# dremovd/PPO

Measured on AMD Instinct MI355X. Metric: env-steps/sec (Pong-shaped synthetic, 256 envs/GPU), higher is better.
Workload: dtype f32

## Files before the change

include/ppo_amd.h:

```cpp
#ifndef PPO_AMD_H
#define PPO_AMD_H

#include <stddef.h>
#include <stdint.h>

#ifdef __cplusplus
extern "C" {
#endif

#define PPO_OK 0
#define PPO_E_INVALID (-1)
#define PPO_E_HIP (-2)
#define PPO_E_ALIGN (-3)

#define PPO_TERM_NONE 0
#define PPO_TERM_U8 1
#define PPO_TERM_F32 2

#define PPO_SCAN_AUTO 0
#define PPO_SCAN_COLUMNS 1
#define PPO_SCAN_TILES 2

int ppo_version(void);
const char *ppo_last_error(void);
// ... 63 lines not shown
    float *dweight;
    float *dbias;
    int n_slabs, cin, cout;
    int accumulate;
} ppo_wgrad_job;
int ppo_conv3x3_backward_weight_slabs_f32(const void *in, int in_mode, const float *dy, void *workspace,
                                          size_t workspace_bytes, int n, int cin, int cout, int h, int w,
                                          int *n_slabs, void *stream);
int ppo_conv3x3_backward_weight_slabs_batch_f32(const void *const *ins, int in_mode, const float *const *dys,
                                                void *const *workspaces, size_t workspace_bytes, int count, int n, int cin,
                                                int cout, int h, int w, int *n_slabs, void *stream);
int ppo_conv3x3_backward_weight_slabs_batch_mixed_f32(const void *const *ins, const int *relu, const float *const *dys,
                                                      void *const *workspaces, size_t workspace_bytes, int count, int n,
                                                      int cin, int cout, int h, int w, int *n_slabs, void *stream);
int ppo_conv3x3_backward_weight_bf16x3_supported(int cin, int cout, int h, int w);
int ppo_conv3x3_backward_weight_slabs_batch_bf16x3(const float *const *ins, const int *relu, const float *const *dys,
                                                   void *const *workspaces, size_t workspace_bytes, int count, int n, int cin,
                                                   int cout, int h, int w, int *n_slabs, void *stream);
int ppo_conv3x3_backward_weight_pooled_supported(int cin, int cout, int h, int w);
int ppo_conv3x3_backward_weight_slabs_pooled_f32(const void *in, int in_mode, const float *g, const uint8_t *argmax,
                                                 void *workspace, size_t workspace_bytes, int n, int cin, int cout, int h,
                                                 int w, int *n_slabs, void *stream);
int ppo_conv3x3_wgrad_reduce_f32(const ppo_wgrad_job *jobs, int n_jobs, void *stream);

int ppo_maxpool3x3s2_forward_f32(const float *in, float *out, uint8_t *argmax, int n, int c, int h, int w,
                                 void *stream);
int ppo_maxpool3x3s2_backward_f32(const float *dout, const uint8_t *argmax, float *din, int n, int c, int h, int w,
                                  void *stream);

size_t ppo_gemm_workspace_bytes(int M, int N, int K);
int ppo_gemm_f32(const float *A, int64_t a_sm, int64_t a_sk, int relu_a, const float *B, int64_t b_sk, int64_t b_sn,
                 int relu_b, const float *bias, const float *mask, float *C, int64_t ldc, int M, int N, int K,
                 void *workspace, size_t workspace_bytes, void *stream);

int ppo_dense_heads_forward_f32(const float *x, int relu_x, const float *W, const float *b, const float *Wh, const float *bh,
                                int relu_h, float *h, float *heads, int M, int K, int H, int NH, void *workspace,
                                size_t workspace_bytes, void *stream);

int ppo_dense_heads_act_forward_f32(const float *x, int relu_x, const float *W, const float *b, const float *Wh,
                                    const float *bh, int relu_h, float *h, float *heads, int M, int K, int H, int NH,
                                    void *workspace, size_t workspace_bytes, int n_actions, float temperature,
                                    uint64_t seed, uint64_t offset, float *log_policy, int32_t *actions, float *log_pac,
                                    float *raw_policy, float *values, int n_value_heads, void *stream);
int ppo_dense_heads_loss_forward_f32(const float *x, int relu_x, const float *W, const float *b, const float *Wh, const float *bh,
                                     int relu_h, float *h, float *heads, int M, int K, int H, int NH, void *workspace,
                                     size_t workspace_bytes, int n_actions, int n_value_heads, const int32_t *actions,
                                     const float *old_log_pac, const float *old_log_policy, const float *advantages,
                                     const float *returns, float eps_clip, float ent_coef, float vf_coef, float grad_scale,
                                     float *dheads, float *stats, const int32_t *index, void *stream);

int ppo_heads_backward_f32(const float *dheads, const float *hin, int relu_in, const float *gate, const float *Wh, float *dh,
                           float *dWh, float *dbh, float *db_next, int B, int H, int NH, void *stream);
int ppo_colsum_f32(const float *X, int M, int N, int64_t ldx, float *out, int accumulate, void *stream);

int ppo_policy_act_f32(const float *heads, int B, int ldo, int n_actions, float temperature, const float *uniform,
                       uint64_t seed, uint64_t offset, int greedy, float *log_policy, int32_t *actions,
                       float *log_pac, float *raw_policy, float *values, int n_value_heads, void *stream);

int ppo_ppo_loss_f32(const float *heads, int B, int ldo, int n_actions, int n_value_heads, const int32_t *actions,
                     const float *old_log_pac, const float *old_log_policy, const float *advantages,
                     const float *returns, float eps_clip, float ent_coef, float vf_coef, float grad_scale,
                     float *dheads, float *stats, const int32_t *index, void *stream);

int ppo_tanh_forward_f32(const float *x, float *y, size_t n, void *stream);
int ppo_tanh_backward_f32(const float *dy, const float *y, float *dx, size_t n, void *stream);

int ppo_value_loss_f32(const float *heads, int B, int ldo, int value_col, int n_value_heads, const float *returns,
                       float vf_coef, int tvf_col, int n_tvf, int tvf_stride, const float *tvf_returns,
                       const float *tvf_weights, float tvf_coef, float grad_scale, float *dheads, float *stats,
                       const int32_t *index, float tvf_keep_prob, uint64_t seed, uint64_t offset, void *stream);

int ppo_distil_loss_f32(const float *heads, int B, int ldo, int n_actions, int pred_col, int n_pred, int pred_stride,
                        int vector_targets, const float *targets, const float *weights, const float *old_policy,
                        const float *log_std, float beta, float grad_scale, float *dheads, float *stats,
                        const int32_t *index, void *stream);

int ppo_gaussian_act_f32(const float *heads, int B, int ldo, int n_actions, const float *log_std, const float *normal,
                         uint64_t seed, uint64_t offset, int deterministic, float *actions, float *log_pac,
                         float *raw_policy, float *values, int n_value_heads, void *stream);

int ppo_gaussian_loss_f32(const float *heads, int B, int ldo, int n_actions, int n_value_heads, const float *actions,
                          const float *old_log_pac, const float *advantages, const float *returns,
                          const float *log_std, float eps_clip, float vf_coef, float grad_scale, float *dheads,
                          float *dlog_std_rows, float *stats, const int32_t *index, void *stream);

size_t ppo_adam_workspace_bytes(void);
int ppo_adam_step_f32(float *params, const float *grads, float *exp_avg, float *exp_avg_sq, int64_t n, int64_t step,
                      double lr, double beta1, double beta2, double eps, float max_grad_norm, float grad_div,
                      void *workspace, float *grad_norm_out, void *stream);
int ppo_adam_step_presummed_f32(float *params, const float *grads, float *exp_avg, float *exp_avg_sq, int64_t n,
                                int64_t step, double lr, double beta1, double beta2, double eps, float max_grad_norm,
                                float grad_div, const float *partials, int n_partials, float *grad_norm_out, void *stream);
int ppo_adam_step_scatter_f32(float *params, const float *grads, float *exp_avg, float *exp_avg_sq, int64_t n, int64_t step,
                              double lr, double beta1, double beta2, double eps, float max_grad_norm, float grad_div,
                              void *workspace, float *grad_norm_out, const int32_t *scatter, int64_t n_scatter,
                              float *packed, void *stream);

int ppo_gather_rows(const void *src, int64_t row_bytes, int64_t n_src_rows, const int32_t *index, int n_rows,
                    void *dst, void *stream);

size_t ppo_moments_workspace_bytes(void);
int ppo_moments_f64(const float *x, int64_t n, double *moments, void *workspace, void *stream);
int ppo_normalize_f32(const float *x, int64_t n, const double *moments, float eps, float *out, float *mean_std_out,
                      void *stream);
int ppo_accumulate_f32(float *dst, const float *src, int64_t n, void *stream);
int ppo_mask_mul_f32(float *w, const uint8_t *mask, int64_t n, void *stream);
// ... 141 lines not shown
```

ppo_amd/_lib.py:

```python
import ctypes
import os
import threading

HERE = os.path.dirname(os.path.abspath(__file__))
LIB_PATH = os.environ.get("PPO_AMD_LIB") or os.path.join(HERE, "lib", "libppo_amd.so")

PPO_TERM_NONE, PPO_TERM_U8, PPO_TERM_F32 = 0, 1, 2
PPO_SCAN_AUTO, PPO_SCAN_COLUMNS, PPO_SCAN_TILES = 0, 1, 2
PPO_IN_NONE, PPO_IN_RELU, PPO_IN_U8 = 0, 1, 2

_vp = ctypes.c_void_p
_i = ctypes.c_int
_i64 = ctypes.c_int64
_d = ctypes.c_double
_f = ctypes.c_float
_sz = ctypes.c_size_t
_u64 = ctypes.c_uint64

SIGNATURES = {
    "ppo_version": (_i, []),
    "ppo_last_error": (ctypes.c_char_p, []),
    "ppo_gae_scan_f32": (_i, [_vp, _vp, _vp, _vp, _i, _vp, _vp, _i, _i, _i64, _d, _d, _d, _i, _vp]),
    "ppo_bootstrapped_returns_f32": (_i, [_vp, _vp, _i, _vp, _vp, _d, _vp, _i, _i, _i64, _vp]),
    "ppo_conv3x3_forward_f32": (_i, [_vp, _i, _vp, _vp, _vp, _vp, _i, _i, _i, _i, _i, _vp]),
    "ppo_conv3x3_backward_data_f32": (_i, [_vp, _vp, _vp, _vp, _vp, _i, _i, _i, _i, _i, _vp]),
    "ppo_conv3x3_wgrad_workspace_bytes": (_sz, [_i, _i]),
    "ppo_conv3x3_backward_weight_f32": (_i, [_vp, _i, _vp, _vp, _vp, _vp, _sz, _i, _i, _i, _i, _i, _i, _vp]),
    "ppo_maxpool3x3s2_forward_f32": (_i, [_vp, _vp, _vp, _i, _i, _i, _i, _vp]),
    "ppo_maxpool3x3s2_backward_f32": (_i, [_vp, _vp, _vp, _i, _i, _i, _i, _vp]),
    "ppo_gemm_workspace_bytes": (_sz, [_i, _i, _i]),
    "ppo_gemm_f32": (_i, [_vp, _i64, _i64, _i, _vp, _i64, _i64, _i, _vp, _vp, _vp, _i64, _i, _i, _i, _vp, _sz, _vp]),
    "ppo_colsum_f32": (_i, [_vp, _i, _i, _i64, _vp, _i, _vp]),
    "ppo_heads_backward_f32": (_i, [_vp, _vp, _i, _vp, _vp, _vp, _vp, _vp, _vp, _i, _i, _i, _vp]),
    "ppo_dense_heads_forward_f32": (_i, [_vp, _i, _vp, _vp, _vp, _vp, _i, _vp, _vp, _i, _i, _i, _i, _vp, _sz, _vp]),
    "ppo_dense_heads_act_forward_f32": (_i, [_vp, _i, _vp, _vp, _vp, _vp, _i, _vp, _vp, _i, _i, _i, _i, _vp, _sz, _i, _f, _u64,
                                             _u64, _vp, _vp, _vp, _vp, _vp, _i, _vp]),
    "ppo_dense_heads_loss_forward_f32": (_i, [_vp, _i, _vp, _vp, _vp, _vp, _i, _vp, _vp, _i, _i, _i, _i, _vp, _sz, _i, _i, _vp, _vp, _vp,
                                              _vp, _vp, _f, _f, _f, _f, _vp, _vp, _vp, _vp]),
    "ppo_policy_act_f32": (_i, [_vp, _i, _i, _i, _f, _vp, _u64, _u64, _i, _vp, _vp, _vp, _vp, _vp, _i, _vp]),
    "ppo_gather_rows": (_i, [_vp, _i64, _i64, _vp, _i, _vp, _vp]),
    "ppo_moments_workspace_bytes": (_sz, []),
    "ppo_moments_f64": (_i, [_vp, _i64, _vp, _vp, _vp]),
    "ppo_normalize_f32": (_i, [_vp, _i64, _vp, _f, _vp, _vp, _vp]),
    "ppo_accumulate_f32": (_i, [_vp, _vp, _i64, _vp]),
    "ppo_mask_mul_f32": (_i, [_vp, _vp, _i64, _vp]),
    "ppo_tvf_returns_workspace_bytes": (_sz, [_i, _i, _i, _i, _i]),
    "ppo_tvf_returns_f32": (_i, [_vp, _vp, _vp, _i, _i, _i, _i, _i, _d, _vp, _vp, _vp, _i, _i, _vp, _vp, _vp, _vp, _vp,
                                 _vp, _sz, _vp, _vp]),
    "ppo_synth_env_create": (_vp, [_i, _i64, _u64, _d, _i64, _i]),
    "ppo_synth_env_destroy": (None, [_vp]),
    "ppo_synth_env_reset": (_i, [_vp, _vp]),
    "ppo_synth_env_step": (_i, [_vp, _vp, _vp, _vp, _vp, _vp, _vp, _vp]),
    "ppo_synth_env_step_upload": (_i, [_vp, _vp, _vp, _vp, _vp, _vp, _vp, _vp, _vp, _i, _vp]),
    "ppo_synth_env_get_state": (_i, [_vp, _vp, _vp, _vp]),
    "ppo_synth_env_set_state": (_i, [_vp, _vp, _vp, _vp, _vp]),
    "ppo_ppo_loss_f32": (_i, [_vp, _i, _i, _i, _i, _vp, _vp, _vp, _vp, _vp, _f, _f, _f, _f, _vp, _vp, _vp, _vp]),
    "ppo_conv3x3_pool_forward_f32": (_i, [_vp, _i, _vp, _vp, _vp, _vp, _i, _i, _i, _i, _i, _vp]),
    "ppo_conv3x3_packed_floats": (_sz, [_i, _i, _i]),
    "ppo_conv3x3_pack_weights_f32": (_i, [_vp, _i, _vp]),
    "ppo_conv3x3_forward_packed_f32": (_i, [_vp, _i, _vp, _vp, _vp, _vp, _i, _i, _i, _i, _i, _vp]),
    "ppo_conv3x3_backward_data_packed_f32": (_i, [_vp, _vp, _vp, _vp, _vp, _i, _i, _i, _i, _i, _vp]),
    "ppo_conv3x3_pool_forward_packed_f32": (_i, [_vp, _i, _vp, _vp, _vp, _vp, _i, _i, _i, _i, _i, _vp]),
    "ppo_conv3x3_pool_forward_packed_indexed_f32": (_i, [_vp, _vp, _i, _vp, _vp, _vp, _vp, _i, _i, _i, _i, _i, _vp]),
    "ppo_conv1_pool_form": (_i, [_i]),
    "ppo_conv3x3_block_supported": (_i, [_i, _i, _i]),
    "ppo_conv3x3_block_forward_packed_f32": (_i, [_vp, _vp, _vp, _vp, _vp, _vp, _i, _i, _i, _i, _vp]),
    "ppo_conv3x3_backward_weight_slabs_f32": (_i, [_vp, _i, _vp, _vp, _sz, _i, _i, _i, _i, _i, _vp, _vp]),
    "ppo_conv3x3_backward_weight_pooled_supported": (_i, [_i, _i, _i, _i]),
    "ppo_conv3x3_backward_weight_slabs_pooled_f32": (_i, [_vp, _i, _vp, _vp, _vp, _sz, _i, _i, _i, _i, _i, _vp, _vp]),
    "ppo_conv3x3_backward_weight_slabs_pooled_indexed_f32": (_i, [_vp, _vp, _i, _vp, _vp, _vp, _sz, _i, _i, _i, _i, _i, _vp, _vp]),
    "ppo_conv3x3_backward_weight_slabs_batch_f32": (_i, [_vp, _i, _vp, _vp, _sz, _i, _i, _i, _i, _i, _i, _vp, _vp]),
    "ppo_conv3x3_backward_weight_slabs_batch_mixed_f32": (_i, [_vp, _vp, _vp, _vp, _sz, _i, _i, _i, _i, _i, _i, _vp, _vp]),
    "ppo_conv3x3_backward_weight_bf16x3_supported": (_i, [_i, _i, _i, _i]),
    "ppo_conv3x3_backward_weight_slabs_batch_bf16x3": (_i, [_vp, _vp, _vp, _vp, _sz, _i, _i, _i, _i, _i, _i, _vp, _vp]),
    "ppo_conv3x3_wgrad_reduce_f32": (_i, [_vp, _i, _vp]),
    "ppo_tanh_forward_f32": (_i, [_vp, _vp, _sz, _vp]),
    "ppo_tanh_backward_f32": (_i, [_vp, _vp, _vp, _sz, _vp]),
    "ppo_value_loss_f32": (_i, [_vp, _i, _i, _i, _i, _vp, _f, _i, _i, _i, _vp, _vp, _f, _f, _vp, _vp, _vp, _f, _u64, _u64, _vp]),
    "ppo_distil_loss_f32": (_i, [_vp, _i, _i, _i, _i, _i, _i, _i, _vp, _vp, _vp, _vp, _f, _f, _vp, _vp, _vp, _vp]),
    "ppo_gaussian_act_f32": (_i, [_vp, _i, _i, _i, _vp, _vp, _u64, _u64, _i, _vp, _vp, _vp, _vp, _i, _vp]),
    "ppo_gaussian_loss_f32": (_i, [_vp, _i, _i, _i, _i, _vp, _vp, _vp, _vp, _vp, _f, _f, _f, _vp, _vp, _vp, _vp, _vp]),
    "ppo_impala_stack_tail_supported": (_i, [_i, _i, _i]),
    "ppo_impala_stack_tail_forward_f32": (_i, [_vp, _vp, _vp, _vp, _vp, _vp, _vp, _i, _i, _i, _i, _vp]),
    "ppo_impala_stack_full_supported": (_i, [_i, _i, _i]),
    "ppo_impala_stack_full_backward_f32": (_i, [_vp] * 10 + [_i, _i, _i, _i, _vp]),
    "ppo_impala_stack_chain_forward_f32": (_i, [_vp] * 15 + [_i, _i, _i, _i, _vp]),
# ... 136 lines not shown
```

ppo_amd/csrc/gemm.hip:

```cpp
#include <algorithm>

#include "common.h"
#include "loss_rows.h"
#include "policy_act.h"
#include "mfma.h"

namespace ppo {
namespace {

#ifndef PPO_TUNE_GEMM_BK
#define PPO_TUNE_GEMM_BK 32
#endif
constexpr int BM = 64, BN = 64, BK = PPO_TUNE_GEMM_BK;
constexpr int PITCH_M = 80, PITCH_K = BK + 2;
constexpr int TILE_WORDS = BM * PITCH_K > BK * PITCH_M ? BM * PITCH_K : BK * PITCH_M;

struct GemmArgs {
    const float *A;
    const float *B;
    float *C;
    const float *bias;
    const float *mask;
    int M, N, K;
    int64_t a_sm, a_sk, b_sk, b_sn, ldc;
// ... 77 lines not shown
};
__device__ __forceinline__ TileId tile_of(int id, int gm, int gn, int split)
{
    const int xcd = id % kXcds, slot = id / kXcds;
    TileId t;
    if (split > 1) {
        const int per = (split + kXcds - 1) / kXcds;
        t.z = xcd * per + slot % per;
        const int tile = slot / per;
        t.tn = tile % gn;
        t.tm = tile / gn;
        t.live = t.z < split && t.tm < gm;
    } else if (gn >= gm) {
        t.z = 0;
        t.tm = slot % gm;
        t.tn = xcd + kXcds * (slot / gm);
        t.live = t.tn < gn;
    } else {
        t.z = 0;
        t.tn = slot % gn;
        t.tm = xcd + kXcds * (slot / gn);
        t.live = t.tm < gm;
    }
    return t;
}
inline int tile_grid(int gm, int gn, int split)
{
    if (split > 1) return kXcds * ((split + kXcds - 1) / kXcds) * gm * gn;
    const int lo = gn >= gm ? gm : gn, hi = gn >= gm ? gn : gm;
    return kXcds * ((hi + kXcds - 1) / kXcds) * lo;
}

#ifndef PPO_TUNE_GEMM_DEPTH
#define PPO_TUNE_GEMM_DEPTH 4
#endif
constexpr int DEPTH = PPO_TUNE_GEMM_DEPTH;

#ifdef PPO_TUNE_GEMM_STAMPS
__device__ unsigned long long ppo_gemm_stamps[1024 * 8];
#define PPO_GSTAMP(slot)                                                                          \
    do {                                                                                          \
        unsigned long long t_;                                                                    \
        __builtin_amdgcn_sched_barrier(0);                                                        \
        asm volatile("s_memtime %0\n\ts_waitcnt lgkmcnt(0)" : "=s"(t_)::"memory");               \
        __builtin_amdgcn_sched_barrier(0);                                                        \
        if (threadIdx.x == 0 && blockIdx.x < 1024) ppo_gemm_stamps[blockIdx.x * 8 + (slot)] = t_; \
    } while (0)
#else
#define PPO_GSTAMP(slot)
#endif
static_assert(DEPTH % 2 == 0, "the LDS buffer of a slab is its slot's parity");

template <bool a_kfast, bool b_kfast, bool vec>
__global__ __launch_bounds__(kGemmThreads) void gemm_f32_kernel(GemmArgs p, int gm, int gn)
{
    __shared__ __align__(16) float s_a[2][TILE_WORDS];
    __shared__ __align__(16) float s_b[2][TILE_WORDS];
    const TileId t = tile_of(blockIdx.x, gm, gn, p.split);
    if (!t.live) return;
    const int tid = threadIdx.x;
    const int lane = tid & 63;
    const int wave = tid >> 6;
    const int l15 = lane & 15;
    const int g = lane >> 4;
    const int wm = (wave / (BN / kWaveN)) * 32;
    const int wn = (wave % (BN / kWaveN)) * kWaveN;
    const int m0 = t.tm * BM;
    const int n0 = t.tn * BN;
    const int kbeg = t.z * p.k_per_slice;
    const int kend = min(p.K, kbeg + p.k_per_slice);

    f32x4 acc[2][kNJ];
#pragma unroll
    for (int i = 0; i < 2; ++i)
#pragma unroll
        for (int j = 0; j < kNJ; ++j) acc[i][j] = f32x4{0.f, 0.f, 0.f, 0.f};

    const int nslabs = kbeg < kend ? (kend - kbeg + BK - 1) / BK : 0;
    const int ngroups = (nslabs + DEPTH - 1) / DEPTH;
    const __amdgpu_buffer_rsrc_t bufA = operand_rsrc(p.A), bufB = operand_rsrc(p.B);
    Slab ra[DEPTH], rb[DEPTH];

    auto fetch = [&](int d, int slab) {
        slab_load<a_kfast, vec>(ra[d], bufA, (int)p.a_sm, (int)p.a_sk, m0, p.M, kbeg + slab * BK, kend, tid);
        slab_load<b_kfast, vec>(rb[d], bufB, (int)p.b_sn, (int)p.b_sk, n0, p.N, kbeg + slab * BK, kend, tid);
    };
    auto stage = [&](int d) {
        slab_store(ra[d], s_a[d & 1], a_kfast, p.relu_a, tid);
        slab_store(rb[d], s_b[d & 1], b_kfast, p.relu_b, tid);
        __syncthreads();
    };
    auto multiply = [&](int d) {
        const float *sa = s_a[d & 1], *sb = s_b[d & 1];
        float a[BK / 4][2], b[BK / 4][kNJ];
#pragma unroll
        for (int ks = 0; ks < BK / 4; ++ks) {
#pragma unroll
            for (int i = 0; i < 2; ++i)
                a[ks][i] = a_kfast ? sa[(wm + i * 16 + l15) * PITCH_K + ks * 4 + g]
                                   : sa[(ks * 4 + g) * PITCH_M + wm + i * 16 + l15];
#pragma unroll
            for (int j = 0; j < kNJ; ++j)
                b[ks][j] = b_kfast ? sb[(wn + j * 16 + l15) * PITCH_K + ks * 4 + g]
                                   : sb[(ks * 4 + g) * PITCH_M + wn + j * 16 + l15];
        }
        __builtin_amdgcn_sched_barrier(0);
#pragma unroll
        for (int ks = 0; ks < BK / 4; ++ks)
#pragma unroll
            for (int i = 0; i < 2; ++i)
#pragma unroll
                for (int j = 0; j < kNJ; ++j) acc[i][j] = mfma16(a[ks][i], b[ks][j], acc[i][j]);
// ... 39 lines not shown
            for (int q = 0; q < kPasses; ++q) {
                const int m = m0 + row0 + kRowsPerPass * q;
                const int off = (m < p.M && col_in) ? (m * (int)p.ldc + n0 + col) * 4 : kOutside;
                gate[q] = buffer_f32x4(bufM, off);
            }
        }
        if (finish && p.bias && col_in) bias4 = *reinterpret_cast<const float4 *>(p.bias + n0 + col);
        __syncthreads();
#pragma unroll
        for (int i = 0; i < 2; ++i)
#pragma unroll
            for (int j = 0; j < kNJ; ++j)
#pragma unroll
                for (int r = 0; r < 4; ++r)
                    sc[(wm + i * 16 + g * 4 + r) * PITCH_C + wn + j * 16 + l15] = acc[i][j][r];
        __syncthreads();
#pragma unroll
        for (int q = 0; q < kPasses; ++q) {
            const int row = row0 + kRowsPerPass * q, m = m0 + row;
            float4 v = *reinterpret_cast<const float4 *>(sc + row * PITCH_C + col);
            if (finish) {
                v.x += bias4.x, v.y += bias4.y, v.z += bias4.z, v.w += bias4.w;
                if (p.mask) {
                    v.x = gate[q].x > 0.f ? v.x : 0.f;
                    v.y = gate[q].y > 0.f ? v.y : 0.f;
                    v.z = gate[q].z > 0.f ? v.z : 0.f;
                    v.w = gate[q].w > 0.f ? v.w : 0.f;
                }
            }
            if (m < p.M && col_in) *reinterpret_cast<float4 *>(C + m * ldc + n0 + col) = v;
        }
    } else {
#pragma unroll
        for (int i = 0; i < 2; ++i)
#pragma unroll
            for (int j = 0; j < kNJ; ++j)
#pragma unroll
                for (int r = 0; r < 4; ++r) {
                    const int m = m0 + wm + i * 16 + g * 4 + r;
                    const int n = n0 + wn + j * 16 + l15;
                    if (m < p.M && n < p.N) {
                        float v = acc[i][j][r];
                        if (finish) {
                            if (p.bias) v += p.bias[n];
                            if (p.mask) v = p.mask[m * p.ldc + n] > 0.f ? v : 0.f;
                        }
                        C[m * ldc + n] = v;
                    }
                }
    }
    PPO_GSTAMP(4);
}

__global__ __launch_bounds__(256) void gemm_finalize_kernel(const float *__restrict__ partial, int split, int M, int N,
                                                            const float *__restrict__ bias,
                                                            const float *__restrict__ mask, float *__restrict__ C,
                                                            int64_t ldc)
{
    const int idx = blockIdx.x * blockDim.x + threadIdx.x;
    if (idx >= M * N) return;
    const int m = idx / N, n = idx % N;
    float v = 0.f;
    const size_t stride = (size_t)M * N;
    int s = 0;
    for (; s + 8 <= split; s += 8) {
        float t[8];
#pragma unroll
        for (int u = 0; u < 8; ++u) t[u] = partial[(size_t)(s + u) * stride + idx];
#pragma unroll
        for (int u = 0; u < 8; ++u) v += t[u];
    }
    for (; s < split; ++s) v += partial[(size_t)s * stride + idx];
    if (bias) v += bias[n];
    if (mask) v = mask[m * ldc + n] > 0.f ? v : 0.f;
    C[m * ldc + n] = v;
}

constexpr int kRowsMaxN = 32, kRowsMaxKPerLane = 8;

template <int NB, int KPL>
__global__ __launch_bounds__(256) void gemm_rows_kernel(GemmArgs p)
{
    const int lane = threadIdx.x & 63;
    const int m = blockIdx.x * 4 + __builtin_amdgcn_readfirstlane(threadIdx.x >> 6);
    if (m >= p.M) return;
    const __amdgpu_buffer_rsrc_t bufA = operand_rsrc(p.A), bufB = operand_rsrc(p.B);
    bool kin[KPL];
#pragma unroll
    for (int i = 0; i < KPL; ++i) kin[i] = lane + 64 * i < p.K;
    float av[KPL];
#pragma unroll
    for (int i = 0; i < KPL; ++i) {
        const int off = kin[i] ? (m * (int)p.a_sm + lane + 64 * i) * 4 : kOutside;
        av[i] = buffer_f32(bufA, off);
    }
    for (int n0 = 0; n0 < p.N; n0 += NB) {
        float bv[NB][KPL];
#pragma unroll
        for (int j = 0; j < NB; ++j) {
            const int row = min(n0 + j, p.N - 1) * (int)p.b_sn;
#pragma unroll
            for (int i = 0; i < KPL; ++i) {
                const int off = kin[i] ? (row + lane + 64 * i) * 4 : kOutside;
                bv[j][i] = buffer_f32(bufB, off);
            }
        }
// ... 21 lines not shown
            if (p.mask) v = p.mask[m * p.ldc + n] > 0.f ? v : 0.f;
            p.C[m * p.ldc + n] = v;
        }
    }
}

__global__ __launch_bounds__(256) void gemm_small_kernel(GemmArgs p)
{
    __shared__ float s[256];
    const int o = blockIdx.x * 16 + (threadIdx.x & 15);
    const int part = threadIdx.x >> 4;
    const bool live = o < p.M * p.N;
    const int m = live ? o / p.N : 0, n = live ? o - m * p.N : 0;
    const float *a = p.A + m * p.a_sm;
    const float *b = p.B + n * p.b_sn;
    const int per = (p.K + 15) / 16;
    const int k0 = part * per, k1 = min(p.K, k0 + per);
    float acc = 0.f;
    if (live) {
        int k = k0;
        for (; k + 8 <= k1; k += 8) {
            float av[8], bv[8];
#pragma unroll
            for (int u = 0; u < 8; ++u) {
                av[u] = a[(k + u) * p.a_sk];
                bv[u] = b[(k + u) * p.b_sk];
            }
#pragma unroll
            for (int u = 0; u < 8; ++u) {
                if (p.relu_a) av[u] = fmaxf(av[u], 0.f);
                if (p.relu_b) bv[u] = fmaxf(bv[u], 0.f);
                acc = fmaf(av[u], bv[u], acc);
            }
        }
        for (; k < k1; ++k) {
            float a0 = a[k * p.a_sk], b0 = b[k * p.b_sk];
            if (p.relu_a) a0 = fmaxf(a0, 0.f);
            if (p.relu_b) b0 = fmaxf(b0, 0.f);
            acc = fmaf(a0, b0, acc);
        }
    }
    s[threadIdx.x] = acc;
    __syncthreads();
    if (part == 0 && live) {
        float v = 0.f;
#pragma unroll
        for (int q = 0; q < 16; ++q) v += s[q * 16 + threadIdx.x];
        if (p.bias) v += p.bias[n];
        if (p.mask) v = p.mask[m * p.ldc + n] > 0.f ? v : 0.f;
        p.C[m * p.ldc + n] = v;
    }
}

__global__ __launch_bounds__(256) void colsum_kernel(const float *__restrict__ X, int M, int N, int64_t ldx,
                                                     float *__restrict__ out, int accumulate)
{
    __shared__ float s[256];
    const int n = blockIdx.x * 16 + (threadIdx.x & 15);
    const int part = threadIdx.x >> 4;
    float v = 0.f;
    if (n < N) {
        for (int m = part; m < M; m += 16 * 8) {
            float t[8];
#pragma unroll
            for (int u = 0; u < 8; ++u) {
                const int mm = m + 16 * u;
                t[u] = mm < M ? X[mm * ldx + n] : 0.f;
            }
#pragma unroll
            for (int u = 0; u < 8; ++u) v += t[u];
        }
    }
    s[threadIdx.x] = v;
    __syncthreads();
    if (part == 0 && n < N) {
        float t = 0.f;
#pragma unroll
        for (int q = 0; q < 16; ++q) t += s[q * 16 + threadIdx.x];
        out[n] = accumulate ? out[n] + t : t;
    }
}

struct ActTail {
    float temperature;
    uint64_t seed, offset;
    ActOut out;
    int loss;
    PpoLossP lp;
    float *dheads;
    const int32_t *index;
};

template <int KPL, int NA, int NHT>
__global__ __launch_bounds__(256) void finalize_heads_kernel(const float *__restrict__ partial, int split, int M, int H,
                                                            const float *__restrict__ bias, float *__restrict__ h,
                                                            const float *__restrict__ Wh, const float *__restrict__ bh, int NH,
                                                            int relu_h, float *__restrict__ heads, ActTail act)
{
    const int lane = threadIdx.x & 63;
    const int m = blockIdx.x * 4 + __builtin_amdgcn_readfirstlane(threadIdx.x >> 6);
    if (m >= M) return;
    const __amdgpu_buffer_rsrc_t pb = buffer_of(partial), wb = buffer_of(Wh), bb = buffer_of(bias, bias != nullptr);
    const int stride = M * H;
    int off[KPL];
#pragma unroll
    for (int i = 0; i < KPL; ++i) off[i] = lane + 64 * i < H ? m * H + lane + 64 * i : -1;
    float bv[NHT][KPL];
#pragma unroll
    for (int j = 0; j < NHT; ++j) {
        const int row = min(j, NH - 1) * H;
#pragma unroll
        for (int i = 0; i < KPL; ++i) bv[j][i] = buffer_f32(wb, off[i] < 0 ? kOutside : (row + lane + 64 * i) * 4);
    }
    float hv[KPL];
#pragma unroll
    for (int i = 0; i < KPL; ++i) hv[i] = 0.f;
    float bsv[KPL];
#pragma unroll
    for (int i = 0; i < KPL; ++i) bsv[i] = buffer_f32(bb, off[i] < 0 ? kOutside : (lane + 64 * i) * 4);
    int s = 0;
    for (; s + 16 <= split; s += 16) {
        float t[KPL][16];
#pragma unroll
        for (int i = 0; i < KPL; ++i)
#pragma unroll
            for (int u = 0; u < 16; ++u) t[i][u] = buffer_f32(pb, off[i] < 0 ? kOutside : ((s + u) * stride + off[i]) * 4);
#pragma unroll
        for (int i = 0; i < KPL; ++i)
#pragma unroll
            for (int u = 0; u < 16; ++u) hv[i] += t[i][u];
    }
    for (; s + 8 <= split; s += 8) {
// ... 125 lines not shown
    }
#pragma unroll
    for (int j = 0; j < 16; ++j) s_red[j][tid] = dW[j];
    s_red[16][tid] = dbn;
    s_red[17][tid] = dbj;
    __syncthreads();
    if (part == 0) {
        float tot[18];
#pragma unroll
        for (int v = 0; v < 18; ++v) {
            float t = 0.f;
#pragma unroll
            for (int q = 0; q < 16; ++q) t += s_red[v][q * 16 + kk];
            tot[v] = t;
        }
        if (col) {
#pragma unroll
            for (int j = 0; j < 16; ++j)
                if (j < a.NH) a.dWh[j * a.H + k] = tot[j];
            if (a.db_next) a.db_next[k] = tot[16];
        }
        if ((int)blockIdx.x == a.xb && a.dbh && kk < a.NH) a.dbh[kk] = tot[17];
    }
}

inline bool vec_ok(const float *P, int64_t s_tile, int64_t s_k, int tile_extent, int k_extent)
{
    const int64_t other = s_k == 1 ? s_tile : s_k;
    const int extent = s_k == 1 ? k_extent : tile_extent;
    return (s_k == 1 || s_tile == 1) && other % 4 == 0 && extent % 4 == 0 && aligned(P, 16);
}

}
}

extern "C" size_t ppo_gemm_workspace_bytes(int M, int N, int K)
{
    (void)K;
    return (size_t)32 * M * N * sizeof(float);
}

namespace ppo {
namespace {
struct HeadsTail {
    const float *Wh, *bh;
    float *heads;
    int NH, relu_h;
    bool fused;
    const ActTail *act = nullptr;
    int act_n = 0;
    bool act_fused = false;
};

int gemm_dispatch(const float *A, int64_t a_sm, int64_t a_sk, int relu_a, const float *B, int64_t b_sk, int64_t b_sn,
                  int relu_b, const float *bias, const float *mask, float *C, int64_t ldc, int M, int N, int K,
                  void *workspace, size_t workspace_bytes, void *stream, HeadsTail *tail)
{
    if (M < 0 || N < 0 || K < 0) return fail(PPO_E_INVALID, "ppo_gemm_f32: negative dimension");
    if (M == 0 || N == 0) return PPO_OK;
    if (!A || !B || !C) return fail(PPO_E_INVALID, "ppo_gemm_f32: null pointer");
    if (ldc < N) return fail(PPO_E_INVALID, "ppo_gemm_f32: ldc < N");
    const int64_t a_last = (int64_t)(M - 1) * a_sm + (int64_t)(K - 1) * a_sk, b_last = (int64_t)(N - 1) * b_sn + (int64_t)(K - 1) * b_sk;
    if (K > 0 && (a_last * 4 + 16 > (int64_t)kBufferBytes || b_last * 4 + 16 > (int64_t)kBufferBytes || a_sm < 0 || a_sk < 0 ||
                  b_sn < 0 || b_sk < 0))
        return fail(PPO_E_INVALID, "ppo_gemm_f32: operand spans 2 GiB or more (or a negative stride); split the batch");
    hipStream_t st = as_stream(stream);
    if ((N <= 16 || K <= 16 || (M <= 16 && a_sm == 1)) && (int64_t)M * N <= (1 << 22)) {
        GemmArgs q{A, B, C, bias, mask, M, N, K, a_sm, a_sk, b_sk, b_sn, ldc, relu_a, relu_b, K, 1, 0, 0, 0};
        if (N <= kRowsMaxN && a_sk == 1 && b_sk == 1 && K <= 64 * kRowsMaxKPerLane) {
            if (K <= 256 && N <= 16)
                hipLaunchKernelGGL((gemm_rows_kernel<16, 4>), dim3((M + 3) / 4), dim3(256), 0, st, q);
            else if (K <= 256)
                hipLaunchKernelGGL((gemm_rows_kernel<8, 4>), dim3((M + 3) / 4), dim3(256), 0, st, q);
            else
                hipLaunchKernelGGL((gemm_rows_kernel<4, kRowsMaxKPerLane>), dim3((M + 3) / 4), dim3(256), 0, st, q);
            return check_launch("gemm_rows_kernel");
        }
        hipLaunchKernelGGL(gemm_small_kernel, dim3((M * N + 15) / 16), dim3(256), 0, st, q);
        return check_launch("gemm_small_kernel");
    }
    const int gm = (M + BM - 1) / BM, gn = (N + BN - 1) / BN;
    constexpr int kSliceK = 256;
    int split = 1;
    const bool few = gn * 4 <= 32;
    if (few && K >= 2 * kSliceK) split = std::min(32, (K + kSliceK - 1) / kSliceK);
    if (split > 1 && (!workspace || workspace_bytes < (size_t)split * M * N * sizeof(float))) split = 1;
    int kps = (K + split - 1) / split;
    kps = (kps + BK - 1) / BK * BK;
    if (split > 1) split = (K + kps - 1) / kps;
    GemmArgs p{A, B, split > 1 ? static_cast<float *>(workspace) : C, bias, mask, M, N, K, a_sm, a_sk, b_sk, b_sn,
               ldc, relu_a, relu_b, kps, split, vec_ok(A, a_sm, a_sk, M, K) ? 1 : 0, vec_ok(B, b_sn, b_sk, N, K) ? 1 : 0, 0};
    p.vec_c = N % 4 == 0 && ldc % 4 == 0 && aligned(C, 16) && aligned(p.C, 16) && (!bias || aligned(bias, 16)) &&
              (!mask || (aligned(mask, 16) && (int64_t)M * ldc * 4 < (int64_t)kBufferBytes));
    const dim3 grid(tile_grid(gm, gn, split));
    const bool vec = p.vec_a && p.vec_b;
    const int variant = (a_sk == 1 ? 4 : 0) | (b_sk == 1 ? 2 : 0) | (vec ? 1 : 0);
#define PPO_GEMM_CASE(v, ak, bk, vc)                                                                  \
    case v:                                                                                           \
        hipLaunchKernelGGL((gemm_f32_kernel<ak, bk, vc>), grid, dim3(kGemmThreads), 0, st, p, gm, gn); \
        break;
    switch (variant) {
        PPO_GEMM_CASE(0, false, false, false)
        PPO_GEMM_CASE(1, false, false, true)
        PPO_GEMM_CASE(2, false, true, false)
        PPO_GEMM_CASE(3, false, true, true)
        PPO_GEMM_CASE(4, true, false, false)
        PPO_GEMM_CASE(5, true, false, true)
        PPO_GEMM_CASE(6, true, true, false)
        PPO_GEMM_CASE(7, true, true, true)
    }
#undef PPO_GEMM_CASE
    int rc = check_launch("gemm_f32_kernel");
    if (rc) return rc;
    if (split > 1) {
        if (tail && !mask && ldc == N && N <= 256 && tail->NH <= 32 && (int64_t)split * M * N * 4 < (int64_t)kBufferBytes) {
#define PPO_FINALIZE(NA, NHT, ACT)                                                                                     \
    hipLaunchKernelGGL((finalize_heads_kernel<4, NA, NHT>), dim3((M + 3) / 4), dim3(256), 0, st,                       \
                       static_cast<const float *>(workspace), split, M, N, bias, C, tail->Wh, tail->bh, tail->NH,      \
                       tail->relu_h, tail->heads, ACT)
            tail->act_fused = tail->act != nullptr;
            const bool wide = tail->NH > 16;
#define PPO_FIN2(NA, ACT)                       \
    do {                                        \
        if (wide) PPO_FINALIZE(NA, 32, ACT);    \
        else PPO_FINALIZE(NA, 16, ACT);         \
    } while (0)
            switch (tail->act ? tail->act_n : 0) {
                case 4: PPO_FIN2(4, *tail->act); break;
                case 6: PPO_FIN2(6, *tail->act); break;
                case 15: PPO_FIN2(15, *tail->act); break;
                case 18: PPO_FIN2(18, *tail->act); break;
                default: PPO_FIN2(0, ActTail{}); tail->act_fused = false;
            }
#undef PPO_FIN2
#undef PPO_FINALIZE
            tail->fused = true;
            return check_launch("finalize_heads_kernel");
        }
        hipLaunchKernelGGL(gemm_finalize_kernel, dim3((M * N + 255) / 256), dim3(256), 0, st,
                           static_cast<const float *>(workspace), split, M, N, bias, mask, C, ldc);
        rc = check_launch("gemm_finalize_kernel");
    }
    return rc;
}
}
}
// ... 60 lines not shown

extern "C" int ppo_dense_heads_loss_forward_f32(const float *x, int relu_x, const float *W, const float *b, const float *Wh,
                                                const float *bh, int relu_h, float *h, float *heads, int M, int K, int H,
                                                int NH, void *workspace, size_t workspace_bytes, int n_actions,
                                                int n_value_heads, const int32_t *actions, const float *old_log_pac,
                                                const float *old_log_policy, const float *advantages, const float *returns,
                                                float eps_clip, float ent_coef, float vf_coef, float grad_scale, float *dheads,
                                                float *stats, const int32_t *index, void *stream)
{
    using namespace ppo;
    if (M < 0 || K < 0 || H <= 0 || NH <= 0) return fail(PPO_E_INVALID, "ppo_dense_heads_loss_forward_f32: bad dimension");
    if (n_actions <= 0 || n_actions > kMaxActions || n_value_heads < 0 || NH < n_actions + n_value_heads)
        return fail(PPO_E_INVALID, "ppo_dense_heads_loss_forward_f32: bad head layout (n_actions=%d value heads=%d of %d)",
                    n_actions, n_value_heads, NH);
    if (M == 0) return PPO_OK;
    if (!x || !W || !Wh || !h || !heads || !actions || !old_log_pac || !advantages || !dheads || (n_value_heads > 0 && !returns))
        return fail(PPO_E_INVALID, "ppo_dense_heads_loss_forward_f32: null pointer");
    ActTail act{};
    act.loss = 1;
    act.lp = PpoLossP{NH, n_actions, n_value_heads, actions, old_log_pac, old_log_policy, advantages, returns, eps_clip,
                      ent_coef, vf_coef, grad_scale, stats};
    act.dheads = dheads, act.index = index;
    HeadsTail tail{Wh, bh, heads, NH, relu_h, false};
    tail.act = &act;
    tail.act_n = n_actions;
    int rc = gemm_dispatch(x, K, 1, relu_x, W, 1, K, 0, b, nullptr, h, H, M, H, K, workspace, workspace_bytes, stream, &tail);
    if (rc) return rc;
    if (!tail.fused)
        rc = gemm_dispatch(h, H, 1, relu_h, Wh, 1, H, 0, bh, nullptr, heads, NH, M, NH, H, nullptr, 0, stream, nullptr);
    if (rc || tail.act_fused) return rc;
    return ppo_ppo_loss_f32(heads, M, NH, n_actions, n_value_heads, actions, old_log_pac, old_log_policy, advantages, returns,
                            eps_clip, ent_coef, vf_coef, grad_scale, dheads, stats, index, stream);
}

extern "C" int ppo_heads_backward_f32(const float *dheads, const float *hin, int relu_in, const float *gate, const float *Wh,
                                      float *dh, float *dWh, float *dbh, float *db_next, int B, int H, int NH, void *stream)
{
    using namespace ppo;
    if (B <= 0 || H <= 0 || NH <= 0 || NH > 16) return fail(PPO_E_INVALID, "ppo_heads_backward_f32: needs B, H > 0 and 1 <= NH <= 16");
    if (!dheads || !hin || !Wh || !dh || !dWh) return fail(PPO_E_INVALID, "ppo_heads_backward_f32: null pointer");
    if ((int64_t)B * H * 4 + 16 > (int64_t)kBufferBytes) return fail(PPO_E_INVALID, "ppo_heads_backward_f32: B * H spans 2 GiB; split the batch");
    HeadsBwdArgs a{dheads, hin, gate, Wh, dh, dWh, dbh, db_next, B, H, NH, relu_in, (B + 3) / 4};
    hipLaunchKernelGGL(heads_backward_kernel, dim3(a.xb + (H + 15) / 16), dim3(256), 0, as_stream(stream), a);
    return check_launch("heads_backward_kernel");
}

extern "C" int ppo_colsum_f32(const float *X, int M, int N, int64_t ldx, float *out, int accumulate, void *stream)
{
    using namespace ppo;
    if (M < 0 || N <= 0 || !X || !out) return fail(PPO_E_INVALID, "ppo_colsum_f32: bad arguments");
    hipLaunchKernelGGL(colsum_kernel, dim3((N + 15) / 16), dim3(256), 0, as_stream(stream), X, M, N, ldx, out, accumulate);
    return check_launch("colsum_kernel");
}
```

ppo_amd/models.py:

```python
import ctypes
import math
import os
from collections import OrderedDict
from typing import Dict, Optional

import numpy as np
import torch

from . import _lib

IN_NONE, IN_RELU, IN_U8 = _lib.PPO_IN_NONE, _lib.PPO_IN_RELU, _lib.PPO_IN_U8
_ALIGN = 4
FUSE_POOL_STACKS = int(os.environ.get("PPO_AMD_FUSE_POOL", "7"))
WGRAD_SIDE_STREAM = int(os.environ.get("PPO_AMD_WGRAD_STREAM", "0"))
WGRAD_BATCH_REDUCE = int(os.environ.get("PPO_AMD_WGRAD_BATCH_REDUCE", "1"))
WGRAD_BATCH_LAUNCH = int(os.environ.get("PPO_AMD_WGRAD_BATCH_LAUNCH", "1"))
WGRAD_POOLED_DY = int(os.environ.get("PPO_AMD_WGRAD_POOLED_DY", "1"))
WGRAD_RIDE = int(os.environ.get("PPO_AMD_WGRAD_RIDE", "1"))
SPLIT_WGRAD = int(os.environ.get("PPO_AMD_SPLIT_WGRAD", "1"))
SPLIT_CONV = int(os.environ.get("PPO_AMD_SPLIT_CONV", "1"))
SPLIT_CONV_POOL = int(os.environ.get("PPO_AMD_SPLIT_CONV_POOL", "1"))
SPLIT_SIGNS = int(os.environ.get("PPO_AMD_SPLIT_SIGNS", "1"))
PACKED_WEIGHTS = int(os.environ.get("PPO_AMD_PACKED_WEIGHTS", "1"))
ADAM_SCATTER = int(os.environ.get("PPO_AMD_ADAM_SCATTER", "0"))
# ... 474 lines not shown
            rec, self._rec = self._rec, None
            try:
                if self._pack_table is not None:
                    self._call("ppo_conv3x3_pack_weights_f32", ctypes.addressof(self._pack_table), len(self._pack_table))
                if self.split_bf16:
                    self._call("ppo_impala_stack_tail_pack_bf16x3_jobs", ctypes.addressof(self._split_jobs), len(self._split_jobs))
                    if self._split_conv_jobs is not None:
                        self._call("ppo_conv3x3_pack_bf16x3_jobs", ctypes.addressof(self._split_conv_jobs), len(self._split_conv_jobs))
            finally:
                self._rec = rec

    def load_state_dict(self, sd, strict=True):
        self.mark_weights_changed()
        missing = [n for n in self.params if n not in sd]
        unexpected = [n for n in sd if n not in self.params]
        if strict and (missing or unexpected):
            raise KeyError(f"state_dict mismatch: missing {missing}, unexpected {unexpected}")
        with torch.no_grad():
            for n, t in sd.items():
                if n in self.params:
                    self.params[n].copy_(torch.as_tensor(t).to(self.device, torch.float32).reshape(self.params[n].shape))
        self.mask_feature_weights()

    def _buf(self, name, shape, dtype=torch.float32):
        key = (name, tuple(shape), dtype)
        t = self._bufs.get(key)
        if t is None:
            t = torch.empty(shape, dtype=dtype, device=self.device)
            self._bufs[key] = t
        return t

    def _ws(self, name, nbytes):
        return self._buf(name, ((nbytes + 3) // 4,), torch.float32)

    def _call(self, fn_name, *args):
        fn = getattr(self.lib, fn_name)
        if self._rec is not None:
            self._rec.append((fn, fn_name, args))
        rc = fn(*args, _lib.current_stream())
        if rc != 0:
            _lib.check(rc, fn_name)

    def _linear(self, x, k, wname, out, relu_x=0, tag=""):
        w = self.params[wname + ".weight"]
        B, n = x.shape[0], w.shape[0]
        ws_bytes = self.lib.ppo_gemm_workspace_bytes(B, n, k)
        ws = self._ws("gemm_ws" + tag, ws_bytes)
        self._call("ppo_gemm_f32", _p(x), k, 1, relu_x, _p(w), 1, k, 0, _p(self.params[wname + ".bias"]), None,
                   _p(out), n, B, n, k, _p(ws), ws_bytes)

    def _linear_backward(self, x, k, wname, dy, dx, relu_x=0, mask=None, acc=0, side=None):
        w = self.params[wname + ".weight"]
        B, n = dy.shape[0], w.shape[0]

        def param_grads():
            self._call("ppo_gemm_f32", _p(dy), 1, n, 0, _p(x), k, 1, relu_x, None, None,
                       _p(self.grads[wname + ".weight"]), k, n, k, B, None, 0)
            if not (wname == "encoder.dense" and getattr(self, "_dense_bias_done", False)):
                self._call("ppo_colsum_f32", _p(dy), B, n, n, _p(self.grads[wname + ".bias"]), acc)

        if side is None:
            param_grads()
        else:
            with torch.cuda.stream(side):
                param_grads()
        if dx is not None:
            self._call("ppo_gemm_f32", _p(dy), n, 1, 0, _p(w), k, 1, 0, None, _p(mask), _p(dx), k, B, k, n, None, 0)

    def _conv(self, x, mode, wname, out, residual, n, cin, cout, h, w):
        pk = self._pk.get((wname, 0))
        if pk is not None:
            self._call("ppo_conv3x3_forward_packed_f32", _p(x), mode, _p(pk), _p(self.params[wname + ".bias"]),
                       _p(residual), _p(out), n, cin, cout, h, w)
            return
        self._call("ppo_conv3x3_forward_f32", _p(x), mode, _p(self.params[wname + ".weight"]),
                   _p(self.params[wname + ".bias"]), _p(residual), _p(out), n, cin, cout, h, w)

    def encode(self, x: torch.Tensor, train: bool, tag: Optional[str] = None):
        sp = self.spec
        tag = tag or ("t" if train else "i")
        self._refresh_packed()
        if tuple(x.shape[1:]) != sp.input_dims:
            raise ValueError(f"expected input [B, {sp.input_dims}], got {tuple(x.shape)}")
        if x.dtype not in (torch.uint8, torch.float32) or not x.is_contiguous() or x.device != self.device:
            raise ValueError("input must be a contiguous uint8/float32 tensor on the model's device")
        key = (tag, x.shape[0], x.dtype, self.allow_chain_split)
        plan = None if train or not self.use_plans else self._plans.get(key)
        if plan is not None:
            calls, acts, x_slots = plan
            st, xp = _lib.current_stream(), x.data_ptr()
            for k, (fn, fn_name, args) in enumerate(calls):
                if self.act_tail is not None and fn_name == "ppo_dense_heads_forward_f32":
                    fn_name, tail, self.act_tail = "ppo_dense_heads_act_forward_f32", self.act_tail, None
                    rc = self.lib.ppo_dense_heads_act_forward_f32(*args, *tail, st)
                else:
                    rc = fn(xp, *args[1:], st) if k in x_slots else fn(*args, st)
                if rc != 0:
                    _lib.check(rc, fn_name)
            out = dict(acts)
            if self.obs_norm is None:
                for name in plan_input_keys(self.encoder_kind):
                    out[name] = x
            return out
        if not train and self.use_plans:
            self._rec = []
        try:
            x_in = x
            if self.obs_norm is not None:
                x_in = self._buf(tag + "xn", tuple(x.shape))
                self._call("ppo_obs_normalize_f32", _p(x), 1 if x.dtype == torch.uint8 else 0, _p(self.obs_norm.mu),
                           _p(self.obs_norm.std), self.obs_norm.norm_eps, _p(x_in), x.shape[0], self.obs_norm.F)
# ... 932 lines not shown
```

Baseline: 97530.

## Fuse dense-layer backward weight grad, bias colsum and input grad into one launch

Adds a combined dense backward kernel that runs the dW GEMM tiles, dx GEMM tiles and bias column-sum blocks in one grid, partitioned by block index. The goal is to cut two kernel launches per dense layer backward and let the three independent pieces share the GPU concurrently. The trade-offs are no split-K for the fused GEMMs, which may underfill the GPU when the reduction dimension is large, and a launch-bounds hint of four blocks that may limit registers. The fused path is used only when no side stream is requested and the shapes are not skinny.

```diff
diff --git a/include/ppo_amd.h b/include/ppo_amd.h
--- a/include/ppo_amd.h
+++ b/include/ppo_amd.h
@@ -139,6 +139,10 @@
 int ppo_heads_backward_f32(const float *dheads, const float *hin, int relu_in, const float *gate, const float *Wh, float *dh,
                            float *dWh, float *dbh, float *db_next, int B, int H, int NH, void *stream);
 int ppo_colsum_f32(const float *X, int M, int N, int64_t ldx, float *out, int accumulate, void *stream);
+
+int ppo_dense_backward_supported(int B, int K, int H);
+int ppo_dense_backward_f32(const float *dy, const float *x, int relu_x, const float *W, const float *mask, float *dW,
+                           float *db, int db_accumulate, float *dx, int B, int K, int H, void *stream);
 
 int ppo_policy_act_f32(const float *heads, int B, int ldo, int n_actions, float temperature, const float *uniform,
                        uint64_t seed, uint64_t offset, int greedy, float *log_policy, int32_t *actions,
diff --git a/ppo_amd/_lib.py b/ppo_amd/_lib.py
--- a/ppo_amd/_lib.py
+++ b/ppo_amd/_lib.py
@@ -32,6 +32,8 @@
     "ppo_gemm_f32": (_i, [_vp, _i64, _i64, _i, _vp, _i64, _i64, _i, _vp, _vp, _vp, _i64, _i, _i, _i, _vp, _sz, _vp]),
     "ppo_colsum_f32": (_i, [_vp, _i, _i, _i64, _vp, _i, _vp]),
     "ppo_heads_backward_f32": (_i, [_vp, _vp, _i, _vp, _vp, _vp, _vp, _vp, _vp, _i, _i, _i, _vp]),
+    "ppo_dense_backward_supported": (_i, [_i, _i, _i]),
+    "ppo_dense_backward_f32": (_i, [_vp, _vp, _i, _vp, _vp, _vp, _vp, _i, _vp, _i, _i, _i, _vp]),
     "ppo_dense_heads_forward_f32": (_i, [_vp, _i, _vp, _vp, _vp, _vp, _i, _vp, _vp, _i, _i, _i, _i, _vp, _sz, _vp]),
     "ppo_dense_heads_act_forward_f32": (_i, [_vp, _i, _vp, _vp, _vp, _vp, _i, _vp, _vp, _i, _i, _i, _i, _vp, _sz, _i, _f, _u64,
                                              _u64, _vp, _vp, _vp, _vp, _vp, _i, _vp]),
diff --git a/ppo_amd/csrc/gemm.hip b/ppo_amd/csrc/gemm.hip
--- a/ppo_amd/csrc/gemm.hip
+++ b/ppo_amd/csrc/gemm.hip
@@ -153,12 +153,8 @@
 static_assert(DEPTH % 2 == 0, "the LDS buffer of a slab is its slot's parity");
 
 template <bool a_kfast, bool b_kfast, bool vec>
-__global__ __launch_bounds__(kGemmThreads) void gemm_f32_kernel(GemmArgs p, int gm, int gn)
-{
-    __shared__ __align__(16) float s_a[2][TILE_WORDS];
-    __shared__ __align__(16) float s_b[2][TILE_WORDS];
-    const TileId t = tile_of(blockIdx.x, gm, gn, p.split);
-    if (!t.live) return;
+__device__ __forceinline__ void gemm_tile(const GemmArgs &p, const TileId t, float (*s_a)[TILE_WORDS], float (*s_b)[TILE_WORDS])
+{
     const int tid = threadIdx.x;
     const int lane = tid & 63;
     const int wave = tid >> 6;
@@ -304,6 +300,16 @@
     PPO_GSTAMP(4);
 }
 
+template <bool a_kfast, bool b_kfast, bool vec>
+__global__ __launch_bounds__(kGemmThreads) void gemm_f32_kernel(GemmArgs p, int gm, int gn)
+{
+    __shared__ __align__(16) float s_a[2][TILE_WORDS];
+    __shared__ __align__(16) float s_b[2][TILE_WORDS];
+    const TileId t = tile_of(blockIdx.x, gm, gn, p.split);
+    if (!t.live) return;
+    gemm_tile<a_kfast, b_kfast, vec>(p, t, s_a, s_b);
+}
+
 __global__ __launch_bounds__(256) void gemm_finalize_kernel(const float *__restrict__ partial, int split, int M, int N,
                                                             const float *__restrict__ bias,
                                                             const float *__restrict__ mask, float *__restrict__ C,
@@ -431,32 +437,66 @@
     }
 }
 
+__device__ __forceinline__ void colsum_block(const float *__restrict__ X, int M, int N, int64_t ldx, float *__restrict__ out,
+                                             int accumulate, int block, float *s, bool active)
+{
+    const int n = block * 16 + (threadIdx.x & 15);
+    const int part = threadIdx.x >> 4;
+    if (active) {
+        float v = 0.f;
+        if (n < N) {
+            for (int m = part; m < M; m += 16 * 8) {
+                float t[8];
+#pragma unroll
+                for (int u = 0; u < 8; ++u) {
+                    const int mm = m + 16 * u;
+                    t[u] = mm < M ? X[mm * ldx + n] : 0.f;
+                }
+#pragma unroll
+                for (int u = 0; u < 8; ++u) v += t[u];
+            }
+        }
+        s[threadIdx.x] = v;
+    }
+    __syncthreads();
+    if (active && part == 0 && n < N) {
+        float t = 0.f;
+#pragma unroll
+        for (int q = 0; q < 16; ++q) t += s[q * 16 + threadIdx.x];
+        out[n] = accumulate ? out[n] + t : t;
+    }
+}
+
 __global__ __launch_bounds__(256) void colsum_kernel(const float *__restrict__ X, int M, int N, int64_t ldx,
                                                      float *__restrict__ out, int accumulate)
 {
     __shared__ float s[256];
-    const int n = blockIdx.x * 16 + (threadIdx.x & 15);
-    const int part = threadIdx.x >> 4;
-    float v = 0.f;
-    if (n < N) {
-        for (int m = part; m < M; m += 16 * 8) {
-            float t[8];
-#pragma unroll
-            for (int u = 0; u < 8; ++u) {
-                const int mm = m + 16 * u;
-                t[u] = mm < M ? X[mm * ldx + n] : 0.f;
-            }
-#pragma unroll
-            for (int u = 0; u < 8; ++u) v += t[u];
-        }
-    }
-    s[threadIdx.x] = v;
-    __syncthreads();
-    if (part == 0 && n < N) {
-        float t = 0.f;
-#pragma unroll
-        for (int q = 0; q < 16; ++q) t += s[q * 16 + threadIdx.x];
-        out[n] = accumulate ? out[n] + t : t;
+    colsum_block(X, M, N, ldx, out, accumulate, blockIdx.x, s, true);
+}
+
+struct DenseBwdArgs {
+    GemmArgs dw, dx;
+    int gm_w, gn_w, grid_w, gm_x, gn_x, grid_x;
+    const float *cs_x;
+    float *cs_out;
+    int cs_m, cs_n, cs_accumulate;
+};
+
+template <bool vec_w, bool vec_x>
+__global__ __launch_bounds__(kGemmThreads, 4) void dense_backward_kernel(DenseBwdArgs a)
+{
+    __shared__ __align__(16) float s_a[2][TILE_WORDS];
+    __shared__ __align__(16) float s_b[2][TILE_WORDS];
+    const int id = blockIdx.x;
+    if (id < a.grid_w) {
+        const TileId t = tile_of(id, a.gm_w, a.gn_w, 1);
+        if (t.live) gemm_tile<false, false, vec_w>(a.dw, t, s_a, s_b);
+    } else if (id < a.grid_w + a.grid_x) {
+        const TileId t = tile_of(id - a.grid_w, a.gm_x, a.gn_x, 1);
+        if (t.live) gemm_tile<true, false, vec_x>(a.dx, t, s_a, s_b);
+    } else {
+        colsum_block(a.cs_x, a.cs_m, a.cs_n, a.cs_n, a.cs_out, a.cs_accumulate, id - a.grid_w - a.grid_x, &s_a[0][0],
+                     threadIdx.x < 256);
     }
 }
 
@@ -688,6 +728,29 @@
     bool act_fused = false;
 };
 
+inline bool skinny(int M, int N, int K, int64_t a_sm)
+{
+    return (N <= 16 || K <= 16 || (M <= 16 && a_sm == 1)) && (int64_t)M * N <= (1 << 22);
+}
+
+inline bool operands_in_range(int M, int N, int K, int64_t a_sm, int64_t a_sk, int64_t b_sk, int64_t b_sn)
+{
+    const int64_t a_last = (int64_t)(M - 1) * a_sm + (int64_t)(K - 1) * a_sk, b_last = (int64_t)(N - 1) * b_sn + (int64_t)(K - 1) * b_sk;
+    return !(K > 0 && (a_last * 4 + 16 > (int64_t)kBufferBytes || b_last * 4 + 16 > (int64_t)kBufferBytes || a_sm < 0 || a_sk < 0 ||
+                       b_sn < 0 || b_sk < 0));
+}
+
+inline GemmArgs tile_args(const float *A, int64_t a_sm, int64_t a_sk, int relu_a, const float *B, int64_t b_sk, int64_t b_sn,
+                          int relu_b, const float *bias, const float *mask, float *C, float *out, int64_t ldc, int M, int N,
+                          int K, int kps, int split)
+{
+    GemmArgs p{A, B, out, bias, mask, M, N, K, a_sm, a_sk, b_sk, b_sn,
+               ldc, relu_a, relu_b, kps, split, vec_ok(A, a_sm, a_sk, M, K) ? 1 : 0, vec_ok(B, b_sn, b_sk, N, K) ? 1 : 0, 0};
+    p.vec_c = N % 4 == 0 && ldc % 4 == 0 && aligned(C, 16) && aligned(p.C, 16) && (!bias || aligned(bias, 16)) &&
+              (!mask || (aligned(mask, 16) && (int64_t)M * ldc * 4 < (int64_t)kBufferBytes));
+    return p;
+}
+
 int gemm_dispatch(const float *A, int64_t a_sm, int64_t a_sk, int relu_a, const float *B, int64_t b_sk, int64_t b_sn,
                   int relu_b, const float *bias, const float *mask, float *C, int64_t ldc, int M, int N, int K,
                   void *workspace, size_t workspace_bytes, void *stream, HeadsTail *tail)
@@ -696,12 +759,10 @@
     if (M == 0 || N == 0) return PPO_OK;
     if (!A || !B || !C) return fail(PPO_E_INVALID, "ppo_gemm_f32: null pointer");
     if (ldc < N) return fail(PPO_E_INVALID, "ppo_gemm_f32: ldc < N");
-    const int64_t a_last = (int64_t)(M - 1) * a_sm + (int64_t)(K - 1) * a_sk, b_last = (int64_t)(N - 1) * b_sn + (int64_t)(K - 1) * b_sk;
-    if (K > 0 && (a_last * 4 + 16 > (int64_t)kBufferBytes || b_last * 4 + 16 > (int64_t)kBufferBytes || a_sm < 0 || a_sk < 0 ||
-                  b_sn < 0 || b_sk < 0))
+    if (!operands_in_range(M, N, K, a_sm, a_sk, b_sk, b_sn))
         return fail(PPO_E_INVALID, "ppo_gemm_f32: operand spans 2 GiB or more (or a negative stride); split the batch");
     hipStream_t st = as_stream(stream);
-    if ((N <= 16 || K <= 16 || (M <= 16 && a_sm == 1)) && (int64_t)M * N <= (1 << 22)) {
+    if (skinny(M, N, K, a_sm)) {
         GemmArgs q{A, B, C, bias, mask, M, N, K, a_sm, a_sk, b_sk, b_sn, ldc, relu_a, relu_b, K, 1, 0, 0, 0};
         if (N <= kRowsMaxN && a_sk == 1 && b_sk == 1 && K <= 64 * kRowsMaxKPerLane) {
             if (K <= 256 && N <= 16)
@@ -724,10 +785,8 @@
     int kps = (K + split - 1) / split;
     kps = (kps + BK - 1) / BK * BK;
     if (split > 1) split = (K + kps - 1) / kps;
-    GemmArgs p{A, B, split > 1 ? static_cast<float *>(workspace) : C, bias, mask, M, N, K, a_sm, a_sk, b_sk, b_sn,
-               ldc, relu_a, relu_b, kps, split, vec_ok(A, a_sm, a_sk, M, K) ? 1 : 0, vec_ok(B, b_sn, b_sk, N, K) ? 1 : 0, 0};
-    p.vec_c = N % 4 == 0 && ldc % 4 == 0 && aligned(C, 16) && aligned(p.C, 16) && (!bias || aligned(bias, 16)) &&
-              (!mask || (aligned(mask, 16) && (int64_t)M * ldc * 4 < (int64_t)kBufferBytes));
+    const GemmArgs p = tile_args(A, a_sm, a_sk, relu_a, B, b_sk, b_sn, relu_b, bias, mask, C,
+                                 split > 1 ? static_cast<float *>(workspace) : C, ldc, M, N, K, kps, split);
     const dim3 grid(tile_grid(gm, gn, split));
     const bool vec = p.vec_a && p.vec_b;
     const int variant = (a_sk == 1 ? 4 : 0) | (b_sk == 1 ? 2 : 0) | (vec ? 1 : 0);
@@ -894,3 +953,41 @@
     hipLaunchKernelGGL(colsum_kernel, dim3((N + 15) / 16), dim3(256), 0, as_stream(stream), X, M, N, ldx, out, accumulate);
     return check_launch("colsum_kernel");
 }
+
+extern "C" int ppo_dense_backward_supported(int B, int K, int H)
+{
+    using namespace ppo;
+    return B > 0 && K > 0 && H > 0 && !skinny(H, K, B, 1) && !skinny(B, K, H, H) && operands_in_range(H, K, B, 1, H, K, 1) &&
+           operands_in_range(B, K, H, H, 1, K, 1);
+}
+
+extern "C" int ppo_dense_backward_f32(const float *dy, const float *x, int relu_x, const float *W, const float *mask, float *dW,
+                                      float *db, int db_accumulate, float *dx, int B, int K, int H, void *stream)
+{
+    using namespace ppo;
+    if (B <= 0 || K <= 0 || H <= 0) return fail(PPO_E_INVALID, "ppo_dense_backward_f32: needs B, K, H > 0");
+    if (!dy || !x || !dW || (dx && !W)) return fail(PPO_E_INVALID, "ppo_dense_backward_f32: null pointer");
+    if (!dx || !ppo_dense_backward_supported(B, K, H)) {
+        int rc = gemm_dispatch(dy, 1, H, 0, x, K, 1, relu_x, nullptr, nullptr, dW, K, H, K, B, nullptr, 0, stream, nullptr);
+        if (rc == PPO_OK && db) rc = ppo_colsum_f32(dy, B, H, H, db, db_accumulate, stream);
+        if (rc == PPO_OK && dx)
+            rc = gemm_dispatch(dy, H, 1, 0, W, K, 1, 0, nullptr, mask, dx, K, B, K, H, nullptr, 0, stream, nullptr);
+        return rc;
+    }
+    const auto whole = [](int k) { return (k + BK - 1) / BK * BK; };
+    DenseBwdArgs a{};
+    a.dw = tile_args(dy, 1, H, 0, x, K, 1, relu_x, nullptr, nullptr, dW, dW, K, H, K, B, whole(B), 1);
+    a.dx = tile_args(dy, H, 1, 0, W, K, 1, 0, nullptr, mask, dx, dx, K, B, K, H, whole(H), 1);
+    a.gm_w = (H + BM - 1) / BM, a.gm_x = (B + BM - 1) / BM, a.gn_w = a.gn_x = (K + BN - 1) / BN;
+    a.grid_w = tile_grid(a.gm_w, a.gn_w, 1), a.grid_x = tile_grid(a.gm_x, a.gn_x, 1);
+    a.cs_x = db ? dy : nullptr, a.cs_out = db, a.cs_m = B, a.cs_n = H, a.cs_accumulate = db_accumulate;
+    const dim3 grid(a.grid_w + a.grid_x + (db ? (H + 15) / 16 : 0));
+    hipStream_t st = as_stream(stream);
+    switch ((a.dw.vec_a && a.dw.vec_b ? 2 : 0) | (a.dx.vec_a && a.dx.vec_b ? 1 : 0)) {
+        case 0: hipLaunchKernelGGL((dense_backward_kernel<false, false>), grid, dim3(kGemmThreads), 0, st, a); break;
+        case 1: hipLaunchKernelGGL((dense_backward_kernel<false, true>), grid, dim3(kGemmThreads), 0, st, a); break;
+        case 2: hipLaunchKernelGGL((dense_backward_kernel<true, false>), grid, dim3(kGemmThreads), 0, st, a); break;
+        default: hipLaunchKernelGGL((dense_backward_kernel<true, true>), grid, dim3(kGemmThreads), 0, st, a); break;
+    }
+    return check_launch("dense_backward_kernel");
+}
diff --git a/ppo_amd/models.py b/ppo_amd/models.py
--- a/ppo_amd/models.py
+++ b/ppo_amd/models.py
@@ -550,11 +550,16 @@
     def _linear_backward(self, x, k, wname, dy, dx, relu_x=0, mask=None, acc=0, side=None):
         w = self.params[wname + ".weight"]
         B, n = dy.shape[0], w.shape[0]
+        bias_done = wname == "encoder.dense" and getattr(self, "_dense_bias_done", False)
+        if side is None and dx is not None and self.lib.ppo_dense_backward_supported(B, k, n):
+            self._call("ppo_dense_backward_f32", _p(dy), _p(x), relu_x, _p(w), _p(mask), _p(self.grads[wname + ".weight"]),
+                       None if bias_done else _p(self.grads[wname + ".bias"]), acc, _p(dx), B, k, n)
+            return
 
         def param_grads():
             self._call("ppo_gemm_f32", _p(dy), 1, n, 0, _p(x), k, 1, relu_x, None, None,
                        _p(self.grads[wname + ".weight"]), k, n, k, B, None, 0)
-            if not (wname == "encoder.dense" and getattr(self, "_dense_bias_done", False)):
+            if not bias_done:
                 self._call("ppo_colsum_f32", _p(dy), B, n, n, _p(self.grads[wname + ".bias"]), acc)
 
         if side is None:
```

Result: no change. 97400 (-0.1%).
